# Ashish424/G.P.U-PathTracer

Measured on AMD Instinct MI355X. Metric: Mrays/sec, cornell_dragon 1920x1080 (+ achieved GB/s against the memory roofline), higher is better.
Workload: dtype f32; 1 GPU; cornell_dragon_800k (800032 tris) 1920x1080 depth 4 diff + reference 8-sphere room, 16 spp per step; kernel=auto, parallelism=1 GPU, closed_scene=True

## Files before the change

### g.p.u-pathtracer_amd/_abi.py

```python
import ctypes as C
import os

_HERE = os.path.dirname(os.path.abspath(__file__))
PTMI_PATH = os.environ.get("PT_LIBPTMI") or os.path.join(_HERE, "csrc", "libptmi.so")
PTHOST_PATH = os.path.join(_HERE, "host", "libpthost.so")


class Camera(C.Structure):
    _fields_ = [("pos", C.c_float * 3), ("front", C.c_float * 3), ("right", C.c_float * 3),
                ("up", C.c_float * 3), ("dist", C.c_float), ("aspect", C.c_float),
                ("fov", C.c_float), ("_pad", C.c_float)]


class Sphere(C.Structure):
    _fields_ = [("pos_rad", C.c_float * 4), ("emi", C.c_float * 3), ("col", C.c_float * 3),
                ("mat", C.c_int32)]


class Material(C.Structure):
    _fields_ = [("col", C.c_float * 3), ("emi", C.c_float * 3), ("mat", C.c_int32), ("phong_expo", C.c_float)]


class DenoiseParams(C.Structure):
    _fields_ = [("width", C.c_int32), ("height", C.c_int32), ("iterations", C.c_int32),
# ... 45 lines not shown
MAT_DIFF, MAT_METAL, MAT_SPEC, MAT_REFR = 0, 1, 2, 3
FLAG_METAL_LITERAL_W = 1 << 0
FLAG_WRITE_RGBA = 1 << 1
FLAG_FACE_FORWARD, FLAG_COSINE_DIFF, FLAG_GLASS_FIX, FLAG_RUSSIAN_ROULETTE, FLAG_MISS_KEEPS_PATH = 1 << 2, 1 << 3, 1 << 4, 1 << 5, 1 << 6
FLAG_RR_CPU_TRACER = 1 << 7
FLAG_NEE = 1 << 8
FLAGS_SMALLPT = FLAG_FACE_FORWARD | FLAG_COSINE_DIFF | FLAG_RUSSIAN_ROULETTE | FLAG_MISS_KEEPS_PATH
FLAGS_CPU_TRACER = FLAG_FACE_FORWARD | FLAG_COSINE_DIFF | FLAG_RR_CPU_TRACER | FLAG_MISS_KEEPS_PATH
RAYS_CLAMPED, RAYS_HDR = 0, 1
ENV_NEAREST, ENV_BILINEAR = 0, 1
KERNEL_AUTO, KERNEL_MEGA_BVH2, KERNEL_PERSISTENT, KERNEL_WAVEFRONT = 0, 1, 3, 5
OPT_KERNEL, OPT_COUNTERS, OPT_TIMING, OPT_BATCH, OPT_TOP_NODES, OPT_OCCUPANCY, OPT_LDS_STACK, OPT_WALK, OPT_LEAF_MAX, OPT_TRI_TEST, OPT_REFILL, OPT_VOTE_NODE, OPT_VOTE_REC, OPT_WAVE_BATCH, OPT_SPHERE_LDS, OPT_BUILD_ALGO, OPT_REBUILD, OPT_PRESPLIT, OPT_WAVE_BLOCKS, OPT_OVERLAP, OPT_OPTIMIZE, OPT_WAVE_SAMPLES = 1, 2, 3, 4, 5, 6, 7, 8, 9, 10, 11, 12, 13, 14, 15, 16, 17, 18, 19, 21, 24, 25
OPT_FIRST_WALK, OPT_PACKET_STACK, OPT_FUSE_STAGES, OPT_LAST_ANYHIT = 26, 27, 28, 29
OPT_ROOT_CULL = 30
OPT_ROOT_ENTRY = 33

_vp, _sz, _i, _u32 = C.c_void_p, C.c_size_t, C.c_int, C.c_uint32
PTMI_SYMBOLS = [
    ("pt_abi_version", _i, []),
    ("pt_device_count", _i, []),
    ("pt_create", _i, [_i, C.POINTER(_vp)]),
    ("pt_destroy", _i, [_vp]),
    ("pt_last_error", C.c_char_p, [_vp]),
    ("pt_set_stream", _i, [_vp, _vp]),
    ("pt_set_option", _i, [_vp, _i, _i]),
    ("pt_sync", _i, [_vp]),
    ("pt_malloc", _i, [_vp, _sz, C.POINTER(_vp)]),
    ("pt_free", _i, [_vp, _vp]),
    ("pt_memset", _i, [_vp, _vp, _i, _sz]),
    ("pt_download", _i, [_vp, _vp, _vp, _sz]),
# ... 97 lines not shown
```

### g.p.u-pathtracer_amd/csrc/pt_ctx.h

```cpp
#pragma once
#include <hip/hip_runtime.h>

#include <algorithm>
#include <climits>
#include <cstdint>
#include <cstring>
#include <string>
#include <type_traits>
#include <vector>

#include "../../include/ptmi.h"
#include "pt_kernels.h"

#ifndef PT_FIRST_WALK_DEFAULT
#define PT_FIRST_WALK_DEFAULT 1
#endif

struct TreeState {
    float4* d_nodes = nullptr;
    bool records_woop = false;
    bool has_bvh = false;
    uint64_t wide_root = 0;
    uint64_t n_wide = 0, n_inner = 0, n_refs = 0, n_leaves = 0, scene_bytes = 0;
    uint32_t wide_top_layout = 0, wide_depth = 0;
// ... 58 lines not shown
    int opt_lstk = 16;
    int opt_walk = 2;
    int opt_leaf_max = 2;
    int opt_tri_test = 0;
    void* d_wave = nullptr;
    size_t wave_bytes = 0;
    int opt_wave_batch = 16;
    int opt_wave_samples = 16;
    int opt_wave_blocks = 8;
    int opt_first_walk = PT_FIRST_WALK_DEFAULT;
    int opt_packet_stack = PT_PACKET_STACK_MAX;
    int opt_fuse_stages = 1;
    int opt_last_anyhit = 1;
    int opt_root_cull = 1;
    int opt_root_entry = 1;
    struct AutoPick {
        static constexpr int TRIALS = 4, PENDING = 4, DECIDED = 5;
        uint64_t key = 0;
        int phase = 0;
        int choice = PT_KERNEL_PERSISTENT;
        hipEvent_t e[2 * TRIALS] = {nullptr, nullptr, nullptr, nullptr, nullptr, nullptr, nullptr, nullptr};
        float ms[2] = {0.f, 0.f};
        uint64_t used = 0;
    };
    static constexpr int N_PICKS = 8;
    AutoPick picks[N_PICKS];
    int pick_last = -1;
    uint64_t pick_tick = 0;
    uint64_t scene_gen = 0;
    uint64_t geom_gen = 0;
// ... 65 lines not shown
}

template <typename K>
hipError_t allow_lds(K kernel, size_t bytes) {
    return hipFuncSetAttribute((const void*)kernel, hipFuncAttributeMaxDynamicSharedMemorySize, (int)bytes);
}

inline bool wide_walk_fits(const TreeState& t, int cap) { return t.has_bvh && 3 * t.wide_depth + 2 <= (uint32_t)cap; }
inline int choose_walk(pt_ctx* c, const char* who, bool postponed) {
    const bool wide_ok = wide_walk_fits(c->tree, PT_STACK_CAP);
    if (c->tree.has_bvh && c->tree.records_woop)
        return wide_ok ? 3 : fail(c, PT_ERR_UNSUPPORTED, std::string(who) + ": Woop records need the wide walk and this tree is too deep for it");
    const int walk = c->opt_walk == 4 && !postponed ? 2 : c->opt_walk;
    return walk >= 2 && !wide_ok ? 1 : walk;
}
inline void scene_view(const pt_ctx* c, KScene& sc, pt_sphere_d* ksph = nullptr) {
    sc = KScene();
    sc.nodes = sc.tris = c->tree.d_nodes;
    sc.has_bvh = c->tree.has_bvh ? 1 : 0;
    sc.wide_root = (int)c->tree.wide_root;
    if (!ksph) return;
    sc.spheres = c->d_spheres; sc.n_spheres = c->n_spheres;
    std::memcpy(ksph, c->h_spheres, sizeof c->h_spheres);
}
inline size_t binary_ray_layout(const pt_ctx* c, KScene& sc) {
    sc.stack_n = PT_STACK_CAP; sc.top_base = 0;
    sc.n_top = (int)std::min<uint32_t>((uint32_t)c->opt_top, c->tree.n_top_layout);
    return lds_fit(sc.n_top, sc.stack_n, PT_BLOCK_RAYS);
}
constexpr size_t QUEUE_BYTES = PT_SHARDS * PT_SHARD_STRIDE * sizeof(unsigned int);
// ... 97 lines not shown
```

### g.p.u-pathtracer_amd/csrc/pt_k_wave.hip

```cpp
#include "pt_ctx.h"

__device__ __forceinline__ int wf_block_rank(bool keep, int& total, int* s_cnt) {
    const unsigned long long m = __ballot(keep);
    const int w = threadIdx.x >> 6;
    const int in_wave = (int)__builtin_amdgcn_mbcnt_hi((uint32_t)(m >> 32), __builtin_amdgcn_mbcnt_lo((uint32_t)m, 0u));
    if ((threadIdx.x & 63) == 0) s_cnt[w] = __popcll(m);
    __syncthreads();
    int base = 0, tot = 0;
#pragma unroll
    for (int k = 0; k < PT_BLOCK / 64; k++) {
        const int c = s_cnt[k];
        if (k < w) base += c;
        tot += c;
    }
    total = tot;
    return base + in_wave;
}

__device__ __forceinline__ void wf_sphere_table() {
    if (threadIdx.x < 11 * PT_KSPHERES) {
        PT_KARGS(K);
        const float v = ((const __attribute__((address_space(4))) float*)&K.ksph[0])[threadIdx.x];
        ((float*)s_dyn)[threadIdx.x] = v;
        if (threadIdx.x % 11 < 4) ((float*)s_dyn)[88 + 4 * (threadIdx.x / 11) + threadIdx.x % 11] = v;
    }
    __syncthreads();
}

__global__ void __launch_bounds__(256) k_wf_prepare(const KParams P) {
    for (uint32_t i = threadIdx.x; i < P.spp; i += 256) P.wf.hashes[i] = pt_wang64(P.frame + i);
    for (uint32_t i = threadIdx.x; i < P.wf.queues_words; i += 256) P.wf.queues_all[i] = 0u;
}

__device__ __forceinline__ bool wf_slot_pixel(const KParams& P, uint32_t slot, uint32_t& s_idx, int& px, int& py) {
    if (slot >= P.wf.n_slots) return false;
    return pt_slot_pixel(P, slot, s_idx, px, py);
}

__device__ __forceinline__ float wf_anyhit_start(float ts) {
    return ts < PT_F32_MAX ? __uint_as_float(__float_as_uint(ts) + 1u) : ts;
}
// ... 160 lines not shown
#ifndef PT_SURVIVOR_RANK
#define PT_SURVIVOR_RANK(P, alive, ps, total, s_cnt) wf_block_rank(alive, total, s_cnt)
#endif

template <bool FIRST>
__device__ __forceinline__ void wf_shade_miss(float* smp, v3 mask) {
    PT_KARGS(K);
    if (FIRST && (K.flags & PT_FLAG_MISS_KEEPS_PATH)) {
        smp[0] = 0.f + mask.x * K.bk[0]; smp[1] = 0.f + mask.y * K.bk[1]; smp[2] = 0.f + mask.z * K.bk[2];
    } else if (K.flags & PT_FLAG_MISS_KEEPS_PATH) {
        smp[0] += mask.x * K.bk[0]; smp[1] += mask.y * K.bk[1]; smp[2] += mask.z * K.bk[2];
    } else {
        smp[0] = K.bk[0]; smp[1] = K.bk[1]; smp[2] = K.bk[2];
    }
}
__device__ __forceinline__ void wf_add_emission(float* smp, v3 e) {
    if (!(e.x == 0.f) || !(e.y == 0.f) || !(e.z == 0.f)) {
        smp[0] += e.x; smp[1] += e.y; smp[2] += e.z;
    }
}

template <bool NEE, bool FIRST, bool LAST>
__device__ __forceinline__ bool wf_shade_segment(const KParams& P, PathState& ps, const Hit& h, bool tri_hit, float* smp, NeeReq* req) {
    v3 tri_n = V3(0.f, 0.f, 0.f);
    if (!LAST && tri_hit) {
        const float4 q3 = P.sc.nodes[h.rec + 3];
        tri_n = V3(q3.x, q3.y, q3.z);
    }
    const SceneHit sh = pt_closest_sphere(P, ps.o, ps.d, h, 0);
    if (sh.geom == 3) {
        wf_shade_miss<FIRST>(smp, ps.mask);
        return false;
    }
    v3 col;
    const bool done = LAST ? true : path_shade_hit(P, ps, h, sh, tri_n, col, 0, NEE ? req : nullptr);
    if (LAST) col = path_last_emission(P, ps, h, sh, 0);
    const v3 e = done ? col : ps.accu;
    if (FIRST) {
        pt_sst3(smp, V3(0.f + e.x, 0.f + e.y, 0.f + e.z));
    } else wf_add_emission(smp, e);
    return !done;
}

template <int LP>
__device__ __forceinline__ void wf_fold_region(const KParams& P, uint32_t region) {
    if (threadIdx.x >= 64) return;
    uint32_t s_idx = 0;
    int px = 0, py = 0;
    const bool in = wf_slot_pixel(P, region * PT_REGION + (threadIdx.x / LP) * (4u * LP), s_idx, px, py);
// ... 33 lines not shown
    total += n_free;
    return walk_free ? n_walk + rf : r;
}

template <bool COUNT>
__device__ __forceinline__ void wf_region_counts(const KParams& P, uint32_t region, int n_walk, int total) {
    if (threadIdx.x != 0) return;
    P.wf.cnt_out[region] = total;
    P.wf.walk_out[region] = n_walk;
    if (COUNT && total != n_walk) {
        atomicAdd(&P.counters[PT_CNT_RAYS], (unsigned long long)(total - n_walk));
        atomicAdd(&P.counters[PT_CNT_WALK_FREE], (unsigned long long)(total - n_walk));
    }
}

template <bool COUNT, bool NEE, bool FIRST, bool LAST = false, int FOLD = 0, bool BOUND = false>
__global__ void __launch_bounds__(PT_BLOCK) k_wf_shade(const KParams P) {
    __shared__ int s_cnt[PT_BLOCK / 64];
    __shared__ int s_cnt2[PT_BLOCK / 64];
    __shared__ int s_cnt_free[PT_BLOCK / 64];
    const uint32_t region = blockIdx.x;
    const int n_in = FIRST ? PT_REGION : P.wf.cnt_in[region];
    const bool last = LAST || P.wf.bounce + 1 >= P.depth;
    if (n_in == 0) {
        if (!last) wf_region_counts<false>(P, region, 0, 0);
        if (NEE && threadIdx.x == 0) P.wf.s_cnt[region] = 0;
        if constexpr (FOLD > 0) wf_fold_region<FOLD>(P, region);
        return;
    }
    wf_sphere_table();
    const size_t i = (size_t)region * PT_REGION + threadIdx.x;
    bool have = (int)threadIdx.x < n_in;
    bool alive = false, tri_hit = false;
    PathState ps;
    NeeReq req;
    req.want = false;
    uint32_t pix = 0, s_idx = 0;
    int px = 0, py = 0;
    if (FIRST) have = wf_slot_pixel(P, (uint32_t)i, s_idx, px, py);
    if (have) {
        if (FIRST) {
            pix = (uint32_t)py * (uint32_t)P.W + (uint32_t)px;
            path_begin_hashed(P, px, py, (uint64_t)pix, P.wf.hashes[s_idx], ps);
        } else {
            const float4 a = pt_sld4(P.wf.ray0_in + i), b = pt_sld4(P.wf.ray1_in + i);
            ps.o = V3(a.x, a.y, a.z);
            ps.d = V3(a.w, b.x, b.y);
            pix = __float_as_uint(b.z);
            ps.nee_mask = 0;
            uint32_t sn = __float_as_uint(b.w);
            if (NEE) {
                ps.nee_mask = (pix >> PT_REC_PIXEL_BITS) | ((sn >> PT_REC_LIGHT_BIT) << 8);
                pix &= (1u << PT_REC_PIXEL_BITS) - 1u;
                sn &= (1u << PT_REC_LIGHT_BIT) - 1u;
            } else if (P.wf.root_entry) sn &= (1u << PT_REC_ENTRY_SHIFT) - 1u;
            s_idx = sn >> PT_REC_DRAW_BITS;
            ps.mask = V3(pt_sld1(P.wf.mask_in + i), pt_sld1(P.wf.mask_in + (size_t)P.wf.cap + i), pt_sld1(P.wf.mask_in + 2 * (size_t)P.wf.cap + i));
            ps.accu = V3(0.f, 0.f, 0.f);
            ps.depth = P.wf.bounce;
            ps.rng = pt_rng_init(P.wf.hashes[s_idx], (uint64_t)pix);
            ps.rng.n = sn & (PT_REC_MAX_DRAWS - 1u);
        }
        const float2 hh = pt_sld2(P.wf.hit + i);
        Hit h;
        h.t = hh.x;
        h.rec = __float_as_int(hh.y);
        h.tri = -1;
        tri_hit = h.t < PT_F32_MAX;
        if (tri_hit) {
            h.tri = 0;
            if (P.tri_matid) h.tri = __float_as_int(P.sc.nodes[h.rec].w);
        }
        alive = wf_shade_segment<NEE, FIRST, LAST>(P, ps, h, tri_hit, pt_sample_ptr(P, s_idx, (size_t)pix), &req);
    }
    float2 bound = make_float2(PT_F32_MAX, __int_as_float(-1));
    if (BOUND && alive) bound = wf_sphere_bound(P, ps);
    if (COUNT) {
        const uint32_t nh = wave_sum_u32(tri_hit ? 1u : 0u), np = wave_sum_u32(have && !alive ? 1u : 0u);
        if ((threadIdx.x & 63) == 0) {
            atomicAdd(&P.counters[PT_CNT_HITS], (unsigned long long)nh);
            atomicAdd(&P.counters[PT_CNT_PATHS], (unsigned long long)np);
        }
    }
    if (NEE) {
        int n_sh;
        const int rs = wf_block_rank(req.want, n_sh, s_cnt2);
        if (req.want) {
            const size_t j = (size_t)region * PT_REGION + (size_t)rs;
// ... 7 lines not shown
        if constexpr (FOLD > 0) {
            __syncthreads();
            wf_fold_region<FOLD>(P, region);
        }
        return;
    }
    int n_walk, total;
    bool walk_free;
    uint32_t entry;
    const int r = wf_survivor_slot<BOUND>(P, alive, ps, bound.x, walk_free, n_walk, total, s_cnt, s_cnt_free, entry);
    if (alive) {
        const size_t j = (size_t)region * PT_REGION + (size_t)r;
        pt_sst4(P.wf.ray0_out + j, make_float4(ps.o.x, ps.o.y, ps.o.z, ps.d.x));
        pt_sst4(P.wf.ray1_out + j, make_float4(ps.d.y, ps.d.z, __uint_as_float(NEE ? (pix | ((ps.nee_mask & 0xffu) << PT_REC_PIXEL_BITS)) : pix),
                                              __uint_as_float((s_idx << PT_REC_DRAW_BITS) | ps.rng.n | (NEE ? (ps.nee_mask >> 8) << PT_REC_LIGHT_BIT : entry))));
        pt_sst1(P.wf.mask_out + j, ps.mask.x);
        pt_sst1(P.wf.mask_out + (size_t)P.wf.cap + j, ps.mask.y);
        pt_sst1(P.wf.mask_out + 2 * (size_t)P.wf.cap + j, ps.mask.z);
        if (BOUND) pt_sst2(P.wf.hit + j, bound);
        else if (walk_free) pt_sst2(P.wf.hit + j, make_float2(pt_no_hit().t, __int_as_float(pt_no_hit().rec)));
    }
    wf_region_counts<COUNT>(P, region, n_walk, total);
}

template <bool COUNT, int FOLD>
__global__ void __launch_bounds__(PT_BLOCK) k_wf_shade_last_any(const KParams P) {
    const uint32_t region = blockIdx.x;
    const int n_in = P.wf.cnt_in[region];
    if (n_in == 0) {
        if constexpr (FOLD > 0) wf_fold_region<FOLD>(P, region);
        return;
    }
    wf_sphere_table();
    const size_t i = (size_t)region * PT_REGION + threadIdx.x;
    const bool have = (int)threadIdx.x < n_in;
    bool tri_hit = false;
    if (have) {
        const float4 b = pt_sld4(P.wf.ray1_in + i);
        const float2 hh = pt_sld2(P.wf.hit + i);
        const v3 mask = V3(pt_sld1(P.wf.mask_in + i), pt_sld1(P.wf.mask_in + (size_t)P.wf.cap + i), pt_sld1(P.wf.mask_in + 2 * (size_t)P.wf.cap + i));
        const uint32_t pix = __float_as_uint(b.z);
        const uint32_t s_idx = (__float_as_uint(b.w) & (P.wf.root_entry ? (1u << PT_REC_ENTRY_SHIFT) - 1u : ~0u)) >> PT_REC_DRAW_BITS;
        float* smp = pt_sample_ptr(P, s_idx, (size_t)pix);
        const int sph = __float_as_int(hh.y);
        tri_hit = hh.x == 0.0f;
        if (!tri_hit && sph >= 0) {
            const float* t = (const float*)s_dyn + 11 * sph;
            wf_add_emission(smp, vadd(V3(0.f, 0.f, 0.f), vmul(mask, V3(t[4], t[5], t[6]))));
        } else if (!tri_hit) {
            wf_shade_miss<false>(smp, mask);
        }
    }
    if (COUNT) {
        const uint32_t nh = wave_sum_u32(tri_hit ? 1u : 0u), np = wave_sum_u32(have ? 1u : 0u);
        if ((threadIdx.x & 63) == 0) {
            atomicAdd(&P.counters[PT_CNT_HITS], (unsigned long long)nh);
            atomicAdd(&P.counters[PT_CNT_PATHS], (unsigned long long)np);
        }
    }
    if constexpr (FOLD > 0) {
        __syncthreads();
        wf_fold_region<FOLD>(P, region);
    }
}

template <bool BOUND>
__global__ void __launch_bounds__(PT_BLOCK, 8) k_wf_extend_packet_shade(const KParams P) {
    __shared__ int s_cnt[PT_BLOCK / 64];
    __shared__ int s_cnt_free[PT_BLOCK / 64];
    wf_sphere_table();
    const uint32_t region = blockIdx.x;
    const size_t i = (size_t)region * PT_REGION + threadIdx.x;
    uint32_t s_idx = 0;
    int px = 0, py = 0;
    const bool have = wf_slot_pixel(P, (uint32_t)i, s_idx, px, py);
    const uint32_t pix = (uint32_t)py * (uint32_t)P.W + (uint32_t)px;
    PathState ps;
    ps.o = ps.d = V3(0.f, 0.f, 0.f);
    if (have) path_begin_hashed(P, px, py, (uint64_t)pix, P.wf.hashes[s_idx], ps);
    TravCount tc;
    Hit h = trav_packet_wide<false>(P.sc, ps.o, ps.d, P.cull != 0, have, tc);
    bool alive = false;
    if (have) {
        const bool tri_hit = h.t < PT_F32_MAX;
        if (tri_hit && !P.tri_matid) h.tri = 0;
        alive = wf_shade_segment<false, true, false>(P, ps, h, tri_hit, pt_sample_ptr(P, s_idx, (size_t)pix), nullptr);
    }
    if (P.wf.bounce + 1 >= P.depth) return;
    float2 bound = make_float2(PT_F32_MAX, __int_as_float(-1));
    if (BOUND && alive) bound = wf_sphere_bound(P, ps);
    int n_walk, total;
    bool walk_free;
    uint32_t entry;
    const int r = wf_survivor_slot<BOUND>(P, alive, ps, bound.x, walk_free, n_walk, total, s_cnt, s_cnt_free, entry);
    if (alive) {
        const size_t j = (size_t)region * PT_REGION + (size_t)r;
        pt_sst4(P.wf.ray0_out + j, make_float4(ps.o.x, ps.o.y, ps.o.z, ps.d.x));
        pt_sst4(P.wf.ray1_out + j, make_float4(ps.d.y, ps.d.z, __uint_as_float(pix), __uint_as_float((s_idx << PT_REC_DRAW_BITS) | ps.rng.n | entry)));
        pt_sst1(P.wf.mask_out + j, ps.mask.x);
        pt_sst1(P.wf.mask_out + (size_t)P.wf.cap + j, ps.mask.y);
        pt_sst1(P.wf.mask_out + 2 * (size_t)P.wf.cap + j, ps.mask.z);
        if (BOUND) pt_sst2(P.wf.hit + j, bound);
        else if (walk_free) pt_sst2(P.wf.hit + j, make_float2(pt_no_hit().t, __int_as_float(pt_no_hit().rec)));
    }
    wf_region_counts<false>(P, region, n_walk, total);
}

__global__ void __launch_bounds__(PT_BLOCK) k_wf_resolve(const KParams P) {
    const int n_in = P.wf.s_cnt[blockIdx.x];
    if ((int)threadIdx.x >= n_in) return;
    const size_t i = (size_t)blockIdx.x * PT_REGION + threadIdx.x;
    const float4 c = P.wf.s_con[i];
    const float2 hh = P.wf.s_hit[i];
    if (hh.x < c.w) return;
    const float4 b = P.wf.s_ray1[i];
    const uint32_t pix = __float_as_uint(b.z), s_idx = __float_as_uint(b.w);
// ... 82 lines not shown
    b.queues = (unsigned int*)base;
    b.nee = base + w.b_q;
    return b;
}

enum WaveExtend { EXT_CLOSEST, EXT_ANY, EXT_FIRST, EXT_PACKET, EXT_FUSED };
enum WaveShade { SHADE_PLAIN, SHADE_BOUND, SHADE_LAST, SHADE_LAST_ANY, SHADE_NONE };
struct WavePlan {
    bool count, nee, deep_stack;
    bool packet;
    bool fuse_first;
    int fold_lp;
    bool anyhit;
    bool root_cull;
    bool root_entry;
    WaveExtend extend(uint32_t b, uint32_t depth) const {
        if (b == 0) return fuse_first ? EXT_FUSED : packet ? EXT_PACKET : EXT_FIRST;
        return anyhit && b + 1 == depth ? EXT_ANY : EXT_CLOSEST;
    }
    WaveShade shade(uint32_t b, uint32_t depth) const {
        if (b == 0 && fuse_first) return SHADE_NONE;
        if (anyhit && b + 1 >= depth) return SHADE_LAST_ANY;
        if (anyhit && b + 2 == depth) return SHADE_BOUND;
        if (b != 0 && !nee && !count && b + 1 >= depth) return SHADE_LAST;
        return SHADE_PLAIN;
    }
};
static WavePlan wave_plan(const pt_ctx* c, const KParams& P, const LaunchCfg& L, bool nee) {
    WavePlan p;
    p.count = L.count; p.nee = nee; p.deep_stack = L.lstk == 24;
    p.packet = c->opt_first_walk == 1 && wide_walk_fits(c->tree, c->opt_packet_stack);
    const bool fuse = c->opt_fuse_stages != 0 && !nee && !L.count, tri_dark = P.tri_emi[0] == 0.f && P.tri_emi[1] == 0.f && P.tri_emi[2] == 0.f;
    p.fuse_first = fuse && p.packet;
    p.fold_lp = fuse && !L.moments && P.depth >= 2 && P.sgroup_log2 >= 2 && P.sgroup_log2 <= 4 && P.spp == (1u << P.sgroup_log2) ? (int)P.spp / 4 : 0;
    p.anyhit = (L.count ? c->opt_last_anyhit == 2 : c->opt_last_anyhit >= 1) && P.depth >= 2 && !nee && !P.tri_matid && tri_dark &&
               P.sc.n_spheres <= PT_KSPHERES && !c->tree.records_woop;
    p.root_cull = L.count ? c->opt_root_cull == 2 : c->opt_root_cull >= 1;
    p.root_entry = p.root_cull && !nee && P.spp < PT_REC_MAX_SAMPLES_ENTRY && (L.count ? c->opt_root_entry == 2 : c->opt_root_entry >= 1);
    return p;
}

constexpr size_t WF_LDS_SHADE = 15 * PT_KSPHERES * 4;
static hipError_t launch_extend(const WavePlan& p, WaveExtend kind, const KParams& Q, const LaunchCfg& L, int blocks_per_cu, hipStream_t s) {
    auto plain = [&](auto kernel, size_t n_blk, size_t lds) {
        hipLaunchKernelGGL(kernel, dim3((unsigned)n_blk), dim3(PT_BLOCK), lds, s, Q);
        return hipGetLastError();
    };
    const size_t n_reg = (size_t)Q.wf.n_regions;
    if (kind == EXT_FUSED)
        return p.anyhit && Q.depth == 2 ? plain(k_wf_extend_packet_shade<true>, n_reg, WF_LDS_SHADE) : plain(k_wf_extend_packet_shade<false>, n_reg, WF_LDS_SHADE);
    if (kind == EXT_PACKET) {
#ifdef PT_PACKET_RESIDENT_GRID
        const bool resident = true;
#else
        const bool resident = p.count;
#endif
        const size_t n_blk = resident ? std::min<size_t>(n_reg, (size_t)8 * L.n_cu) : n_reg;
        return p.count ? plain(k_wf_extend_packet<true>, n_blk, 0) : plain(k_wf_extend_packet<false>, n_blk, 0);
    }
    return with_bool(p.count, [&](auto count) {
        return with_bool(p.deep_stack, [&](auto deep) {
            constexpr int OCC = deep() ? 6 : 8, LSTK = deep() ? 24 : 16;
            auto go = [&](auto first, auto any, auto entry) {
                return launch_resident(k_wf_extend<count(), OCC, LSTK, first(), any(), entry()>, (size_t)LSTK * PT_BLOCK * 4, blocks_per_cu, L.n_cu,
                                       (size_t)Q.wf.n_regions, s, Q);
            };
            if (kind == EXT_FIRST) return go(std::true_type{}, std::false_type{}, std::false_type{});
            return with_bool(p.root_entry, [&](auto entry) {
                if (kind == EXT_ANY) return go(std::false_type{}, std::true_type{}, entry);
                return go(std::false_type{}, std::false_type{}, entry);
            });
        });
    });
}

static hipError_t launch_shade(const WavePlan& p, WaveShade kind, bool first, const KParams& Q, hipStream_t s) {
    auto go = [&](auto kernel) {
        hipLaunchKernelGGL(kernel, dim3((unsigned)Q.wf.n_regions), dim3(PT_BLOCK), WF_LDS_SHADE, s, Q);
        return hipGetLastError();
    };
    if (p.count) {
        if (kind == SHADE_LAST_ANY) return go(k_wf_shade_last_any<true, 0>);
        return with_bool(first, [&](auto f) {
            if (kind == SHADE_BOUND) return go(k_wf_shade<true, false, f(), false, 0, true>);
            return p.nee ? go(k_wf_shade<true, true, f()>) : go(k_wf_shade<true, false, f()>);
        });
    }
    if (kind == SHADE_LAST_ANY) return with_int<4, 2, 1, 0>(p.fold_lp, [&](auto lp) { return go(k_wf_shade_last_any<false, lp()>); });
    if (kind == SHADE_LAST) return with_int<4, 2, 1, 0>(p.fold_lp, [&](auto lp) { return go(k_wf_shade<false, false, false, true, lp()>); });
    return with_bool(first, [&](auto f) {
        if (kind == SHADE_BOUND) return go(k_wf_shade<false, false, f(), false, 0, true>);
        return p.nee ? go(k_wf_shade<false, true, f()>) : go(k_wf_shade<false, false, f()>);
    });
}

int render_wavefront(pt_ctx* c, KParams& P, const LaunchCfg& L, int work_tiles, bool& folded) {
    folded = false;
    WaveLayout w;
    int rc = wave_layout(c, P, work_tiles, w);
    if (rc == PT_OK) rc = wave_reserve(c, w);
    if (rc != PT_OK) return rc;
    const WaveBuffers buf = wave_carve((char*)c->d_wave, w);
    const WavePlan plan = wave_plan(c, P, L, w.nee);
    folded = plan.fold_lp != 0;
    P.wf.nee = w.nee ? 1 : 0;
    P.wf.root_cull = plan.root_cull ? 1 : 0;
    P.wf.root_entry = plan.root_entry ? 1 : 0;
// ... 52 lines not shown
```

### g.p.u-pathtracer_amd/csrc/pt_kernels.h

```cpp
#pragma once
#include "pt_math.h"
#include "pt_env.h"
#include "../../include/ptmi.h"

#define PT_BLOCK 256
#define PT_BLOCK_RAYS 256
#define PT_TILE 8
#define PT_MAX_TOP 1024
#define PT_STACK_CAP 72
#define PT_SHARDS 8
#define PT_SHARD_STRIDE 32
#define PT_REGION 256

struct KScene {
    const float4* __restrict__ nodes;
    const float4* __restrict__ tris;
    const pt_sphere_d* __restrict__ spheres;
    int n_spheres;
    int has_bvh;
    int n_top;
    int stack_n;
    int top_base;
    int wide_root;
};
// ... 22 lines not shown
            bool distinct = true;
            for (uint32_t i = 0; i < n; i++)
                for (uint32_t j = i + 1; j < n; j++) distinct = distinct && c[i] != c[j];
            bool rest_zero = true;
            for (uint32_t i = n; i < 4; i++) rest_zero = rest_zero && c[i] == 0u;
            if (!distinct || !rest_zero) continue;
            const uint32_t code = pt_entry_pack(n, c[0], c[1], c[2]);
            if (code >= (1u << PT_REC_ENTRY_BITS) || pt_entry_count(code) != n) return false;
            for (uint32_t k = 0; k < n; k++)
                if (pt_entry_child(code, k) != c[k]) return false;
            seen++;
        }
    return seen == 64u;
}
static_assert(pt_entry_round_trips(), "the entry code of PT_OPT_ROOT_ENTRY");
struct KWave {
    const float4* __restrict__ ray0_in;
    const float4* __restrict__ ray1_in;
    const float* __restrict__ mask_in;
    float4* __restrict__ ray0_out;
    float4* __restrict__ ray1_out;
    float* __restrict__ mask_out;
    float2* __restrict__ hit;
    const int* __restrict__ walk_in;
    const int* __restrict__ cnt_in;
    int* __restrict__ cnt_out;
    int* __restrict__ walk_out;
    unsigned long long* hashes;
    unsigned int* queue;
    unsigned int* queues_all;
// ... 214 lines not shown
```

### g.p.u-pathtracer_amd/csrc/ptmi.hip

```cpp
#include <hip/hip_runtime.h>

#include <algorithm>
#include <cmath>
#include <cstdio>
#include <cstring>
#include <string>
#include <vector>

#include "pt_ctx.h"

static_assert(sizeof(pt_sphere) == 44, "pt_sphere must match the reference Sphere (44 B)");
static_assert(sizeof(pt_sphere_d) == sizeof(pt_sphere), "device sphere mirror");
static_assert(sizeof(pt_params) == 104 && sizeof(pt_camera) == 64 && sizeof(pt_counters) == 48, "ABI struct sizes (tests/test_host_and_abi.py)");

namespace ptmi {
thread_local std::string g_err;
}
using namespace ptmi;

namespace ptmi {
static bool auto_decide(pt_ctx* c, pt_ctx::AutoPick& a, bool wait) {
    using AP = pt_ctx::AutoPick;
    if (a.phase != AP::PENDING) return a.phase == AP::DECIDED;
    for (int t = 0; t < AP::TRIALS; t++) {
// ... 61 lines not shown
    {PT_OPT_WAVE_BATCH, &pt_ctx::opt_wave_batch, OptionRow::RANGE, {1, 64}, PT_ERR_INVALID, "pt_set_option: wave batch must be 1..64"},
    {PT_OPT_VOTE_NODE, &pt_ctx::opt_vote_node, OptionRow::RANGE, {1, 64}, PT_ERR_INVALID, "pt_set_option: vote weight must be 1..64"},
    {PT_OPT_VOTE_REC, &pt_ctx::opt_vote_rec, OptionRow::RANGE, {1, 64}, PT_ERR_INVALID, "pt_set_option: vote weight must be 1..64"},
    {PT_OPT_OPTIMIZE, &pt_ctx::opt_optimize, OptionRow::RANGE, {0, 16}, PT_ERR_INVALID, "pt_set_option: optimize passes must be 0 (off) .. 16"},
    {PT_OPT_WAVE_SAMPLES, &pt_ctx::opt_wave_samples, OptionRow::RANGE, {1, 64}, PT_ERR_INVALID, "pt_set_option: wave samples must be 1 (one sample of a tile per wave) .. 64"},
    {PT_OPT_WAVE_BLOCKS, &pt_ctx::opt_wave_blocks, OptionRow::RANGE, {1, 8}, PT_ERR_INVALID, "pt_set_option: wave blocks must be 1..8 per CU"},
    {PT_OPT_LDS_STACK, &pt_ctx::opt_lstk, OptionRow::SET, {0, 16, 24, 24}, PT_ERR_INVALID, "pt_set_option: LDS stack must be 0 (all 72 entries in LDS), 16 or 24 entries"},
    {PT_OPT_REFILL, &pt_ctx::opt_refill, OptionRow::RANGE, {1, 64}, PT_ERR_INVALID, "pt_set_option: refill must be 1..64"},
    {PT_OPT_BATCH, &pt_ctx::opt_batch, OptionRow::RANGE, {1, 64}, PT_ERR_INVALID, "pt_set_option: batch must be 1..64"},
    {PT_OPT_FIRST_WALK, &pt_ctx::opt_first_walk, OptionRow::RANGE, {0, 1}, PT_ERR_INVALID, "pt_set_option: first walk must be 0 (per lane) or 1 (wave-wide packets)"},
    {PT_OPT_PACKET_STACK, &pt_ctx::opt_packet_stack, OptionRow::RANGE, {2, PT_PACKET_STACK_MAX}, PT_ERR_INVALID, "pt_set_option: packet stack must be 2..72 entries"},
    {PT_OPT_FUSE_STAGES, &pt_ctx::opt_fuse_stages, OptionRow::RANGE, {0, 1}, PT_ERR_INVALID, "pt_set_option: fuse stages must be 0 (separate launches) or 1"},
    {PT_OPT_LAST_ANYHIT, &pt_ctx::opt_last_anyhit, OptionRow::RANGE, {0, 2}, PT_ERR_INVALID, "pt_set_option: last any-hit must be 0 (off), 1 (product launches) or 2 (instrumented launches too)"},
    {PT_OPT_ROOT_CULL, &pt_ctx::opt_root_cull, OptionRow::RANGE, {0, 2}, PT_ERR_INVALID, "pt_set_option: root cull must be 0 (off), 1 (product launches) or 2 (instrumented launches too)"},
    {PT_OPT_ROOT_ENTRY, &pt_ctx::opt_root_entry, OptionRow::RANGE, {0, 2}, PT_ERR_INVALID, "pt_set_option: root entry must be 0 (off), 1 (product launches) or 2 (instrumented launches too)"},
};
}

extern "C" {

int pt_abi_version(void) { return PTMI_ABI_VERSION; }

int pt_device_count(void) {
    int n = 0;
    hipError_t e = hipGetDeviceCount(&n);
    if (e != hipSuccess) { g_err = std::string("hipGetDeviceCount: ") + hipGetErrorString(e); return PT_ERR_DEVICE; }
    return n;
}

const char* pt_last_error(const pt_ctx* ctx) { return ctx ? ctx->err.c_str() : g_err.c_str(); }
// ... 659 lines not shown
```

### include/ptmi.h

```cpp
#ifndef PTMI_H
#define PTMI_H

#include <stddef.h>
#include <stdint.h>

#ifdef __cplusplus
extern "C" {
#endif

#define PTMI_ABI_VERSION 3

typedef struct pt_ctx pt_ctx;

typedef enum pt_status {
    PT_OK = 0,
    PT_ERR_INVALID = -1,
    PT_ERR_DEVICE = -2,
    PT_ERR_NO_SCENE = -3,
    PT_ERR_NOMEM = -4,
    PT_ERR_UNSUPPORTED = -5
} pt_status;

enum { PT_MAT_DIFF = 0, PT_MAT_METAL = 1, PT_MAT_SPEC = 2, PT_MAT_REFR = 3 };

// ... 34 lines not shown
    PT_OPT_SPHERE_LDS = 15,
    PT_OPT_WAVE_BLOCKS = 19,
    PT_OPT_WAVE_SAMPLES = 25,
    PT_OPT_FIRST_WALK = 26,
    PT_OPT_PACKET_STACK = 27,
    PT_OPT_OVERLAP = 21,
    PT_OPT_BUILD_ALGO = 16,
    PT_OPT_REBUILD = 17,
    PT_OPT_OPTIMIZE = 24,
    PT_OPT_PRESPLIT = 18,
    PT_OPT_TRI_TEST = 10,
    PT_OPT_LEAF_MAX = 9,
    PT_OPT_FUSE_STAGES = 28,
    PT_OPT_LAST_ANYHIT = 29,
    PT_OPT_ROOT_CULL = 30,
    PT_OPT_ROOT_ENTRY = 33
};

typedef struct pt_camera {
    float pos[3];
    float front[3];
    float right[3];
    float up[3];
    float dist;
    float aspect;
    float fov;
    float _pad;
} pt_camera;

typedef struct pt_sphere {
    float pos_rad[4];
// ... 151 lines not shown
```

Measured before the change: 17540 Mrays/s.

## Encode path throughput as a packed hit-history word instead of three mask floats

In the wavefront path, each surviving path now stores one 32-bit word recording the material code (sphere id or triangle) of every bounce, instead of three float mask channels. The shade kernels rebuild mask and accumulated emission by replaying that history against an LDS table of sphere and triangle colours. This is meant to cut per-ray memory traffic in the mask buffers. The cost is a short replay loop per shaded ray. It only applies when the scene has no NEE, no Russian roulette, no refractive materials, no per-triangle materials and limited depth.

```diff
diff --git a/g.p.u-pathtracer_amd/_abi.py b/g.p.u-pathtracer_amd/_abi.py
--- a/g.p.u-pathtracer_amd/_abi.py
+++ b/g.p.u-pathtracer_amd/_abi.py
@@ -83,6 +83,7 @@
 OPT_FIRST_WALK, OPT_PACKET_STACK, OPT_FUSE_STAGES, OPT_LAST_ANYHIT = 26, 27, 28, 29
 OPT_ROOT_CULL = 30
 OPT_ROOT_ENTRY = 33
+OPT_PATH_HISTORY = 34
 
 _vp, _sz, _i, _u32 = C.c_void_p, C.c_size_t, C.c_int, C.c_uint32
 PTMI_SYMBOLS = [
diff --git a/g.p.u-pathtracer_amd/csrc/pt_ctx.h b/g.p.u-pathtracer_amd/csrc/pt_ctx.h
--- a/g.p.u-pathtracer_amd/csrc/pt_ctx.h
+++ b/g.p.u-pathtracer_amd/csrc/pt_ctx.h
@@ -96,6 +96,7 @@
     int opt_last_anyhit = 1;
     int opt_root_cull = 1;
     int opt_root_entry = 1;
+    int opt_path_history = 1;
     struct AutoPick {
         static constexpr int TRIALS = 4, PENDING = 4, DECIDED = 5;
         uint64_t key = 0;
@@ -191,6 +192,14 @@
     const int walk = c->opt_walk == 4 && !postponed ? 2 : c->opt_walk;
     return walk >= 2 && !wide_ok ? 1 : walk;
 }
+inline bool path_history_holds(const KParams& P) {
+    if ((P.flags & (PT_FLAG_NEE | PT_FLAG_RUSSIAN_ROULETTE | PT_FLAG_RR_CPU_TRACER)) || P.tri_matid || P.sc.n_spheres > PT_KSPHERES ||
+        P.tri_mat == PT_MAT_REFR || P.depth > PT_HIST_MAX_DEPTH)
+        return false;
+    for (int i = 0; i < P.sc.n_spheres; i++)
+        if (P.ksph[i].mat == PT_MAT_REFR) return false;
+    return true;
+}
 inline void scene_view(const pt_ctx* c, KScene& sc, pt_sphere_d* ksph = nullptr) {
     sc = KScene();
     sc.nodes = sc.tris = c->tree.d_nodes;
diff --git a/g.p.u-pathtracer_amd/csrc/pt_k_wave.hip b/g.p.u-pathtracer_amd/csrc/pt_k_wave.hip
--- a/g.p.u-pathtracer_amd/csrc/pt_k_wave.hip
+++ b/g.p.u-pathtracer_amd/csrc/pt_k_wave.hip
@@ -17,6 +17,8 @@
     return base + in_wave;
 }
 
+constexpr int WF_TRI_ROW = 15 * PT_KSPHERES - 4;
+template <bool HIST = false>
 __device__ __forceinline__ void wf_sphere_table() {
     if (threadIdx.x < 11 * PT_KSPHERES) {
         PT_KARGS(K);
@@ -24,7 +26,25 @@
         ((float*)s_dyn)[threadIdx.x] = v;
         if (threadIdx.x % 11 < 4) ((float*)s_dyn)[88 + 4 * (threadIdx.x / 11) + threadIdx.x % 11] = v;
     }
+    if (HIST && threadIdx.x >= 128 && threadIdx.x < 134) {
+        PT_KARGS(K);
+        const int k = (int)threadIdx.x - 128;
+        ((float*)s_dyn)[WF_TRI_ROW + (k < 3 ? 7 + k : 1 + k)] = ((const __attribute__((address_space(4))) float*)&K.tri_col[0])[k];
+    }
     __syncthreads();
+}
+
+__device__ __forceinline__ const float* wf_history_row(uint32_t code) {
+    return (const float*)s_dyn + (code == PT_HIST_TRI ? (uint32_t)WF_TRI_ROW : 11u * code);
+}
+__device__ __forceinline__ void wf_history_replay(uint32_t word, uint32_t n, v3& mask, v3& accu) {
+    mask = V3(1.f, 1.f, 1.f);
+    accu = V3(0.f, 0.f, 0.f);
+    for (uint32_t k = 0; k < n; k++) {
+        const float* t = wf_history_row(pt_hist_code(word, k));
+        accu = vadd(accu, vmul(mask, V3(t[4], t[5], t[6])));
+        mask = vmul(mask, V3(t[7], t[8], t[9]));
+    }
 }
 
 __global__ void __launch_bounds__(256) k_wf_prepare(const KParams P) {
@@ -215,14 +235,20 @@
         smp[0] = K.bk[0]; smp[1] = K.bk[1]; smp[2] = K.bk[2];
     }
 }
+__device__ __forceinline__ void wf_shade_miss_history(float* smp, v3 accu, v3 mask) {
+    PT_KARGS(K);
+    if (K.flags & PT_FLAG_MISS_KEEPS_PATH) pt_sst3(smp, V3(accu.x + mask.x * K.bk[0], accu.y + mask.y * K.bk[1], accu.z + mask.z * K.bk[2]));
+    else pt_sst3(smp, V3(K.bk[0], K.bk[1], K.bk[2]));
+}
 __device__ __forceinline__ void wf_add_emission(float* smp, v3 e) {
     if (!(e.x == 0.f) || !(e.y == 0.f) || !(e.z == 0.f)) {
         smp[0] += e.x; smp[1] += e.y; smp[2] += e.z;
     }
 }
 
-template <bool NEE, bool FIRST, bool LAST>
-__device__ __forceinline__ bool wf_shade_segment(const KParams& P, PathState& ps, const Hit& h, bool tri_hit, float* smp, NeeReq* req) {
+template <bool NEE, bool FIRST, bool LAST, bool HIST = false>
+__device__ __forceinline__ bool wf_shade_segment(const KParams& P, PathState& ps, const Hit& h, bool tri_hit, float* smp, NeeReq* req, uint32_t& code) {
+    static_assert(!(NEE && HIST), "k_wf_resolve adds to the sample colour in place");
     v3 tri_n = V3(0.f, 0.f, 0.f);
     if (!LAST && tri_hit) {
         const float4 q3 = P.sc.nodes[h.rec + 3];
@@ -230,10 +256,21 @@
     }
     const SceneHit sh = pt_closest_sphere(P, ps.o, ps.d, h, 0);
     if (sh.geom == 3) {
-        wf_shade_miss<FIRST>(smp, ps.mask);
+        if (HIST) wf_shade_miss_history(smp, ps.accu, ps.mask);
+        else wf_shade_miss<FIRST>(smp, ps.mask);
         return false;
     }
     v3 col;
+    if (HIST) {
+        code = sh.geom == 1 ? (uint32_t)sh.sph_id : PT_HIST_TRI;
+        if (LAST) {
+            pt_sst3(smp, vadd(ps.accu, path_last_emission(P, ps, h, sh, 0)));
+            return false;
+        }
+        const bool ended = path_shade_hit(P, ps, h, sh, tri_n, col, 0, nullptr);
+        if (ended) pt_sst3(smp, FIRST ? V3(0.f + col.x, 0.f + col.y, 0.f + col.z) : col);
+        return !ended;
+    }
     const bool done = LAST ? true : path_shade_hit(P, ps, h, sh, tri_n, col, 0, NEE ? req : nullptr);
     if (LAST) col = path_last_emission(P, ps, h, sh, 0);
     const v3 e = done ? col : ps.accu;
@@ -297,7 +334,7 @@
     }
 }
 
-template <bool COUNT, bool NEE, bool FIRST, bool LAST = false, int FOLD = 0, bool BOUND = false>
+template <bool COUNT, bool NEE, bool FIRST, bool LAST = false, int FOLD = 0, bool BOUND = false, bool HIST = false>
 __global__ void __launch_bounds__(PT_BLOCK) k_wf_shade(const KParams P) {
     __shared__ int s_cnt[PT_BLOCK / 64];
     __shared__ int s_cnt2[PT_BLOCK / 64];
@@ -311,10 +348,11 @@
         if constexpr (FOLD > 0) wf_fold_region<FOLD>(P, region);
         return;
     }
-    wf_sphere_table();
+    wf_sphere_table<HIST>();
     const size_t i = (size_t)region * PT_REGION + threadIdx.x;
     bool have = (int)threadIdx.x < n_in;
     bool alive = false, tri_hit = false;
+    uint32_t hist = 0, code = 0;
     PathState ps;
     NeeReq req;
     req.want = false;
@@ -338,8 +376,13 @@
                 sn &= (1u << PT_REC_LIGHT_BIT) - 1u;
             } else if (P.wf.root_entry) sn &= (1u << PT_REC_ENTRY_SHIFT) - 1u;
             s_idx = sn >> PT_REC_DRAW_BITS;
-            ps.mask = V3(pt_sld1(P.wf.mask_in + i), pt_sld1(P.wf.mask_in + (size_t)P.wf.cap + i), pt_sld1(P.wf.mask_in + 2 * (size_t)P.wf.cap + i));
-            ps.accu = V3(0.f, 0.f, 0.f);
+            if (HIST) {
+                hist = __float_as_uint(pt_sld1(P.wf.mask_in + i));
+                wf_history_replay(hist, P.wf.bounce, ps.mask, ps.accu);
+            } else {
+                ps.mask = V3(pt_sld1(P.wf.mask_in + i), pt_sld1(P.wf.mask_in + (size_t)P.wf.cap + i), pt_sld1(P.wf.mask_in + 2 * (size_t)P.wf.cap + i));
+                ps.accu = V3(0.f, 0.f, 0.f);
+            }
             ps.depth = P.wf.bounce;
             ps.rng = pt_rng_init(P.wf.hashes[s_idx], (uint64_t)pix);
             ps.rng.n = sn & (PT_REC_MAX_DRAWS - 1u);
@@ -354,7 +397,7 @@
             h.tri = 0;
             if (P.tri_matid) h.tri = __float_as_int(P.sc.nodes[h.rec].w);
         }
-        alive = wf_shade_segment<NEE, FIRST, LAST>(P, ps, h, tri_hit, pt_sample_ptr(P, s_idx, (size_t)pix), &req);
+        alive = wf_shade_segment<NEE, FIRST, LAST, HIST>(P, ps, h, tri_hit, pt_sample_ptr(P, s_idx, (size_t)pix), &req, code);
     }
     float2 bound = make_float2(PT_F32_MAX, __int_as_float(-1));
     if (BOUND && alive) bound = wf_sphere_bound(P, ps);
@@ -392,16 +435,19 @@
         pt_sst4(P.wf.ray0_out + j, make_float4(ps.o.x, ps.o.y, ps.o.z, ps.d.x));
         pt_sst4(P.wf.ray1_out + j, make_float4(ps.d.y, ps.d.z, __uint_as_float(NEE ? (pix | ((ps.nee_mask & 0xffu) << PT_REC_PIXEL_BITS)) : pix),
                                               __uint_as_float((s_idx << PT_REC_DRAW_BITS) | ps.rng.n | (NEE ? (ps.nee_mask >> 8) << PT_REC_LIGHT_BIT : entry))));
-        pt_sst1(P.wf.mask_out + j, ps.mask.x);
-        pt_sst1(P.wf.mask_out + (size_t)P.wf.cap + j, ps.mask.y);
-        pt_sst1(P.wf.mask_out + 2 * (size_t)P.wf.cap + j, ps.mask.z);
+        if (HIST) pt_sst1(P.wf.mask_out + j, __uint_as_float(pt_hist_push(hist, P.wf.bounce, code)));
+        else {
+            pt_sst1(P.wf.mask_out + j, ps.mask.x);
+            pt_sst1(P.wf.mask_out + (size_t)P.wf.cap + j, ps.mask.y);
+            pt_sst1(P.wf.mask_out + 2 * (size_t)P.wf.cap + j, ps.mask.z);
+        }
         if (BOUND) pt_sst2(P.wf.hit + j, bound);
         else if (walk_free) pt_sst2(P.wf.hit + j, make_float2(pt_no_hit().t, __int_as_float(pt_no_hit().rec)));
     }
     wf_region_counts<COUNT>(P, region, n_walk, total);
 }
 
-template <bool COUNT, int FOLD>
+template <bool COUNT, int FOLD, bool HIST = false>
 __global__ void __launch_bounds__(PT_BLOCK) k_wf_shade_last_any(const KParams P) {
     const uint32_t region = blockIdx.x;
     const int n_in = P.wf.cnt_in[region];
@@ -409,20 +455,28 @@
         if constexpr (FOLD > 0) wf_fold_region<FOLD>(P, region);
         return;
     }
-    wf_sphere_table();
+    wf_sphere_table<HIST>();
     const size_t i = (size_t)region * PT_REGION + threadIdx.x;
     const bool have = (int)threadIdx.x < n_in;
     bool tri_hit = false;
     if (have) {
         const float4 b = pt_sld4(P.wf.ray1_in + i);
         const float2 hh = pt_sld2(P.wf.hit + i);
-        const v3 mask = V3(pt_sld1(P.wf.mask_in + i), pt_sld1(P.wf.mask_in + (size_t)P.wf.cap + i), pt_sld1(P.wf.mask_in + 2 * (size_t)P.wf.cap + i));
+        v3 mask, accu = V3(0.f, 0.f, 0.f);
+        if (HIST) wf_history_replay(__float_as_uint(pt_sld1(P.wf.mask_in + i)), P.wf.bounce, mask, accu);
+        else mask = V3(pt_sld1(P.wf.mask_in + i), pt_sld1(P.wf.mask_in + (size_t)P.wf.cap + i), pt_sld1(P.wf.mask_in + 2 * (size_t)P.wf.cap + i));
         const uint32_t pix = __float_as_uint(b.z);
         const uint32_t s_idx = (__float_as_uint(b.w) & (P.wf.root_entry ? (1u << PT_REC_ENTRY_SHIFT) - 1u : ~0u)) >> PT_REC_DRAW_BITS;
         float* smp = pt_sample_ptr(P, s_idx, (size_t)pix);
         const int sph = __float_as_int(hh.y);
         tri_hit = hh.x == 0.0f;
-        if (!tri_hit && sph >= 0) {
+        if (HIST) {
+            if (tri_hit) pt_sst3(smp, accu);
+            else if (sph >= 0) {
+                const float* t = (const float*)s_dyn + 11 * sph;
+                pt_sst3(smp, vadd(accu, vadd(V3(0.f, 0.f, 0.f), vmul(mask, V3(t[4], t[5], t[6])))));
+            } else wf_shade_miss_history(smp, accu, mask);
+        } else if (!tri_hit && sph >= 0) {
             const float* t = (const float*)s_dyn + 11 * sph;
             wf_add_emission(smp, vadd(V3(0.f, 0.f, 0.f), vmul(mask, V3(t[4], t[5], t[6]))));
         } else if (!tri_hit) {
@@ -442,11 +496,11 @@
     }
 }
 
-template <bool BOUND>
+template <bool BOUND, bool HIST = false>
 __global__ void __launch_bounds__(PT_BLOCK, 8) k_wf_extend_packet_shade(const KParams P) {
     __shared__ int s_cnt[PT_BLOCK / 64];
     __shared__ int s_cnt_free[PT_BLOCK / 64];
-    wf_sphere_table();
+    wf_sphere_table<HIST>();
     const uint32_t region = blockIdx.x;
     const size_t i = (size_t)region * PT_REGION + threadIdx.x;
     uint32_t s_idx = 0;
@@ -459,10 +513,11 @@
     TravCount tc;
     Hit h = trav_packet_wide<false>(P.sc, ps.o, ps.d, P.cull != 0, have, tc);
     bool alive = false;
+    uint32_t code = 0;
     if (have) {
         const bool tri_hit = h.t < PT_F32_MAX;
         if (tri_hit && !P.tri_matid) h.tri = 0;
-        alive = wf_shade_segment<false, true, false>(P, ps, h, tri_hit, pt_sample_ptr(P, s_idx, (size_t)pix), nullptr);
+        alive = wf_shade_segment<false, true, false, HIST>(P, ps, h, tri_hit, pt_sample_ptr(P, s_idx, (size_t)pix), nullptr, code);
     }
     if (P.wf.bounce + 1 >= P.depth) return;
     float2 bound = make_float2(PT_F32_MAX, __int_as_float(-1));
@@ -475,9 +530,12 @@
         const size_t j = (size_t)region * PT_REGION + (size_t)r;
         pt_sst4(P.wf.ray0_out + j, make_float4(ps.o.x, ps.o.y, ps.o.z, ps.d.x));
         pt_sst4(P.wf.ray1_out + j, make_float4(ps.d.y, ps.d.z, __uint_as_float(pix), __uint_as_float((s_idx << PT_REC_DRAW_BITS) | ps.rng.n | entry)));
-        pt_sst1(P.wf.mask_out + j, ps.mask.x);
-        pt_sst1(P.wf.mask_out + (size_t)P.wf.cap + j, ps.mask.y);
-        pt_sst1(P.wf.mask_out + 2 * (size_t)P.wf.cap + j, ps.mask.z);
+        if (HIST) pt_sst1(P.wf.mask_out + j, __uint_as_float(pt_hist_push(0u, 0u, code)));
+        else {
+            pt_sst1(P.wf.mask_out + j, ps.mask.x);
+            pt_sst1(P.wf.mask_out + (size_t)P.wf.cap + j, ps.mask.y);
+            pt_sst1(P.wf.mask_out + 2 * (size_t)P.wf.cap + j, ps.mask.z);
+        }
         if (BOUND) pt_sst2(P.wf.hit + j, bound);
         else if (walk_free) pt_sst2(P.wf.hit + j, make_float2(pt_no_hit().t, __int_as_float(pt_no_hit().rec)));
     }
@@ -590,6 +648,7 @@
     bool anyhit;
     bool root_cull;
     bool root_entry;
+    bool history;
     WaveExtend extend(uint32_t b, uint32_t depth) const {
         if (b == 0) return fuse_first ? EXT_FUSED : packet ? EXT_PACKET : EXT_FIRST;
         return anyhit && b + 1 == depth ? EXT_ANY : EXT_CLOSEST;
@@ -612,11 +671,12 @@
     p.anyhit = (L.count ? c->opt_last_anyhit == 2 : c->opt_last_anyhit >= 1) && P.depth >= 2 && !nee && !P.tri_matid && tri_dark &&
                P.sc.n_spheres <= PT_KSPHERES && !c->tree.records_woop;
     p.root_cull = L.count ? c->opt_root_cull == 2 : c->opt_root_cull >= 1;
+    p.history = (L.count ? c->opt_path_history == 2 : c->opt_path_history >= 1) && path_history_holds(P);
     p.root_entry = p.root_cull && !nee && P.spp < PT_REC_MAX_SAMPLES_ENTRY && (L.count ? c->opt_root_entry == 2 : c->opt_root_entry >= 1);
     return p;
 }
 
-constexpr size_t WF_LDS_SHADE = 15 * PT_KSPHERES * 4;
+constexpr size_t WF_LDS_SHADE = (15 * PT_KSPHERES + 6) * 4;
 static hipError_t launch_extend(const WavePlan& p, WaveExtend kind, const KParams& Q, const LaunchCfg& L, int blocks_per_cu, hipStream_t s) {
     auto plain = [&](auto kernel, size_t n_blk, size_t lds) {
         hipLaunchKernelGGL(kernel, dim3((unsigned)n_blk), dim3(PT_BLOCK), lds, s, Q);
@@ -624,7 +684,9 @@
     };
     const size_t n_reg = (size_t)Q.wf.n_regions;
     if (kind == EXT_FUSED)
-        return p.anyhit && Q.depth == 2 ? plain(k_wf_extend_packet_shade<true>, n_reg, WF_LDS_SHADE) : plain(k_wf_extend_packet_shade<false>, n_reg, WF_LDS_SHADE);
+        return with_bool(p.history, [&](auto hist) {
+            return p.anyhit && Q.depth == 2 ? plain(k_wf_extend_packet_shade<true, hist()>, n_reg, WF_LDS_SHADE) : plain(k_wf_extend_packet_shade<false, hist()>, n_reg, WF_LDS_SHADE);
+        });
     if (kind == EXT_PACKET) {
 #ifdef PT_PACKET_RESIDENT_GRID
         const bool resident = true;
@@ -655,18 +717,23 @@
         hipLaunchKernelGGL(kernel, dim3((unsigned)Q.wf.n_regions), dim3(PT_BLOCK), WF_LDS_SHADE, s, Q);
         return hipGetLastError();
     };
-    if (p.count) {
-        if (kind == SHADE_LAST_ANY) return go(k_wf_shade_last_any<true, 0>);
+    if (p.nee) return with_bool(p.count, [&](auto count) {
+        return with_bool(first, [&](auto f) { return go(k_wf_shade<count(), true, f()>); });
+    });
+    return with_bool(p.history, [&](auto hist) {
+        if (p.count) {
+            if (kind == SHADE_LAST_ANY) return go(k_wf_shade_last_any<true, 0, hist()>);
+            return with_bool(first, [&](auto f) {
+                if (kind == SHADE_BOUND) return go(k_wf_shade<true, false, f(), false, 0, true, hist()>);
+                return go(k_wf_shade<true, false, f(), false, 0, false, hist()>);
+            });
+        }
+        if (kind == SHADE_LAST_ANY) return with_int<4, 2, 1, 0>(p.fold_lp, [&](auto lp) { return go(k_wf_shade_last_any<false, lp(), hist()>); });
+        if (kind == SHADE_LAST) return with_int<4, 2, 1, 0>(p.fold_lp, [&](auto lp) { return go(k_wf_shade<false, false, false, true, lp(), false, hist()>); });
         return with_bool(first, [&](auto f) {
-            if (kind == SHADE_BOUND) return go(k_wf_shade<true, false, f(), false, 0, true>);
-            return p.nee ? go(k_wf_shade<true, true, f()>) : go(k_wf_shade<true, false, f()>);
+            if (kind == SHADE_BOUND) return go(k_wf_shade<false, false, f(), false, 0, true, hist()>);
+            return go(k_wf_shade<false, false, f(), false, 0, false, hist()>);
         });
-    }
-    if (kind == SHADE_LAST_ANY) return with_int<4, 2, 1, 0>(p.fold_lp, [&](auto lp) { return go(k_wf_shade_last_any<false, lp()>); });
-    if (kind == SHADE_LAST) return with_int<4, 2, 1, 0>(p.fold_lp, [&](auto lp) { return go(k_wf_shade<false, false, false, true, lp()>); });
-    return with_bool(first, [&](auto f) {
-        if (kind == SHADE_BOUND) return go(k_wf_shade<false, false, f(), false, 0, true>);
-        return p.nee ? go(k_wf_shade<false, true, f()>) : go(k_wf_shade<false, false, f()>);
     });
 }
 
diff --git a/g.p.u-pathtracer_amd/csrc/pt_kernels.h b/g.p.u-pathtracer_amd/csrc/pt_kernels.h
--- a/g.p.u-pathtracer_amd/csrc/pt_kernels.h
+++ b/g.p.u-pathtracer_amd/csrc/pt_kernels.h
@@ -60,6 +60,22 @@
     return seen == 64u;
 }
 static_assert(pt_entry_round_trips(), "the entry code of PT_OPT_ROOT_ENTRY");
+constexpr uint32_t PT_HIST_BITS = 4, PT_HIST_TRI = 8, PT_HIST_MAX_DEPTH = 32 / PT_HIST_BITS + 1;
+constexpr uint32_t pt_hist_push(uint32_t word, uint32_t bounce, uint32_t code) { return word | (code << (PT_HIST_BITS * bounce)); }
+constexpr uint32_t pt_hist_code(uint32_t word, uint32_t bounce) { return (word >> (PT_HIST_BITS * bounce)) & ((1u << PT_HIST_BITS) - 1u); }
+constexpr bool pt_hist_round_trips() {
+    for (uint32_t b = 0; b + 1 < PT_HIST_MAX_DEPTH; b++)
+        for (uint32_t code = 0; code <= PT_HIST_TRI; code++) {
+            uint32_t w = 0;
+            for (uint32_t k = 0; k < b; k++) w = pt_hist_push(w, k, (code + k) % (PT_HIST_TRI + 1u));
+            w = pt_hist_push(w, b, code);
+            if (pt_hist_code(w, b) != code) return false;
+            for (uint32_t k = 0; k < b; k++)
+                if (pt_hist_code(w, k) != (code + k) % (PT_HIST_TRI + 1u)) return false;
+        }
+    return PT_HIST_TRI >= PT_KSPHERES && PT_HIST_TRI < (1u << PT_HIST_BITS);
+}
+static_assert(pt_hist_round_trips(), "the history word of PT_OPT_PATH_HISTORY");
 struct KWave {
     const float4* __restrict__ ray0_in;
     const float4* __restrict__ ray1_in;
diff --git a/g.p.u-pathtracer_amd/csrc/ptmi.hip b/g.p.u-pathtracer_amd/csrc/ptmi.hip
--- a/g.p.u-pathtracer_amd/csrc/ptmi.hip
+++ b/g.p.u-pathtracer_amd/csrc/ptmi.hip
@@ -99,6 +99,7 @@
     {PT_OPT_LAST_ANYHIT, &pt_ctx::opt_last_anyhit, OptionRow::RANGE, {0, 2}, PT_ERR_INVALID, "pt_set_option: last any-hit must be 0 (off), 1 (product launches) or 2 (instrumented launches too)"},
     {PT_OPT_ROOT_CULL, &pt_ctx::opt_root_cull, OptionRow::RANGE, {0, 2}, PT_ERR_INVALID, "pt_set_option: root cull must be 0 (off), 1 (product launches) or 2 (instrumented launches too)"},
     {PT_OPT_ROOT_ENTRY, &pt_ctx::opt_root_entry, OptionRow::RANGE, {0, 2}, PT_ERR_INVALID, "pt_set_option: root entry must be 0 (off), 1 (product launches) or 2 (instrumented launches too)"},
+    {PT_OPT_PATH_HISTORY, &pt_ctx::opt_path_history, OptionRow::RANGE, {0, 2}, PT_ERR_INVALID, "pt_set_option: path history must be 0 (off), 1 (product launches) or 2 (instrumented launches too)"},
 };
 }
 
diff --git a/include/ptmi.h b/include/ptmi.h
--- a/include/ptmi.h
+++ b/include/ptmi.h
@@ -72,7 +72,8 @@
     PT_OPT_FUSE_STAGES = 28,
     PT_OPT_LAST_ANYHIT = 29,
     PT_OPT_ROOT_CULL = 30,
-    PT_OPT_ROOT_ENTRY = 33
+    PT_OPT_ROOT_ENTRY = 33,
+    PT_OPT_PATH_HISTORY = 34
 };
 
 typedef struct pt_camera {
```

Result: faster. 18100 Mrays/s, median of 6 (+3.2%).
